# abiswas-odu/Disco

Measured on AMD Instinct MI355X. Metric: overlaps/sec (BuildGraph stage), 150 bp reads, higher is better.
Workload: dtype u64; 1 GPU; 50000000 x 150 bp synthetic reads, 30x of 50 x 5000000 bp uniform-random contigs, both strands, error-free, min-overlap 40 (k=39), transitive reduction on, seed 42; reads=50000000, read_len=150, min_overlap=40, parallelism=1 GPU, e_pre=903537181, e_out=45314794, n_contained=4685156, cap_bind_sites=0, asymmetric_pairs=0, probes=5550000000, kmer_hits=2220071992

## Files before the change

disco_amd/buildgraph.py:

```python
from __future__ import annotations

import ctypes as C
import os

import numpy as np

_HERE = os.path.dirname(os.path.abspath(__file__))
_LIBPATH = os.environ.get("DISCO_LIB") or os.path.join(_HERE, "libdisco_hip.so")
_lib = None


class DiscoError(RuntimeError):
    pass


class Params(C.Structure):
    _fields_ = [("min_overlap", C.c_uint32), ("max_edges_per_kmer", C.c_uint32), ("flags", C.c_uint32), ("max_substitutions", C.c_uint32)]


class GenSpecABI(C.Structure):
    _fields_ = [("seed", C.c_uint64), ("n_reads", C.c_uint64), ("contig_len", C.c_uint64), ("n_contigs", C.c_uint32),
                ("len_min", C.c_uint32), ("len_max", C.c_uint32), ("skew", C.c_uint32)]


# ... 59 lines not shown
    ("disco_contract_chains", C.c_int, [_P, C.c_uint32, C.POINTER(C.c_uint64), C.POINTER(C.c_uint64)]),
    ("disco_contract_chains_of", C.c_int, [_P, _P, C.c_uint64, C.c_uint32, C.POINTER(C.c_uint64), C.POINTER(C.c_uint64)]),
    ("disco_fetch_chains", C.c_int, [_P, _P, _P, _P]),
    ("disco_set_query_order", C.c_int, [_P, _P]),
    ("disco_get_query_order", C.c_int, [_P, C.POINTER(_P)]),
    ("disco_probe_run_words", C.c_int, [_P]),
    ("disco_measure_hbm", C.c_int, [_P, C.c_uint64, C.c_int, C.POINTER(C.c_double)]),
    ("disco_measure_gather", C.c_int, [_P, C.c_uint64, C.c_int, C.POINTER(C.c_double)]),
    ("disco_comm_unique_id", C.c_int, [_P, C.c_size_t]),
    ("disco_comm_init", C.c_int, [_P, _P, C.c_int, C.c_int]),
    ("disco_comm_init_local", C.c_int, [C.POINTER(_P), C.c_int]),
    ("disco_comm_rank", C.c_int, [_P]),
    ("disco_comm_world", C.c_int, [_P]),
    ("disco_comm_kind", C.c_char_p, [_P]),
    ("disco_dist_range", C.c_int, [_P, C.c_uint64, C.POINTER(C.c_uint64), C.POINTER(C.c_uint64)]),
    ("disco_dist_upload_reads", C.c_int, [_P, _P, C.c_uint32, _P, C.c_uint64]),
    ("disco_dist_generate_reads", C.c_int, [_P, C.POINTER(GenSpecABI)]),
    ("disco_dist_run_graph", C.c_int, [_P, C.c_uint32]),
    ("disco_dist_get_info", C.c_int, [_P, _P]),
    ("disco_ingest_fasta", C.c_int, [_P, C.POINTER(C.c_char_p), C.c_int, C.c_uint32, _P, _P]),
    ("disco_ingest_fetch", C.c_int, [_P, _P, _P]),
]

ABI_VERSION = 2
FLAG_TWO_PASS_VERIFY = 1
XCHG = ("reads", "index_records", "index_shards", "contain", "row_requests", "row_data", "push", "adjacency", "twins", "queries", "hits", "keys", "reads_dealt", "contain_keys")
UNIQUE_ID_BYTES = 128
DIST_GATHER_READS = 1
DIST_KEEP_INDEX_PARTITIONED = 2


CHAIN_EDGE_DTYPE = np.dtype([("a", "<u8"), ("b", "<u8"), ("offset", "<u8"), ("orient", "<u4"), ("n_links", "<u4"), ("first_link", "<u8")])
CHAIN_LINK_DTYPE = np.dtype([("to", "<u4"), ("offset", "<u4"), ("orient", "<u4")])


class IngestFile(C.Structure):
    _fields_ = [("first_index", C.c_uint64), ("last_index", C.c_uint64), ("good", C.c_uint64), ("bad", C.c_uint64)]


class IngestInfo(C.Structure):
    _fields_ = [("n_reads", C.c_uint64), ("total_records", C.c_uint64), ("too_long", C.c_uint64), ("stride_words", C.c_uint32), ("shortest", C.c_uint32),
                ("longest", C.c_uint32), ("read_s", C.c_float), ("device_s", C.c_float)]


class DistInfo(C.Structure):
    _fields_ = [("world", C.c_uint32), ("rank", C.c_uint32), ("n_reads", C.c_uint64), ("own_lo", C.c_uint64), ("own_hi", C.c_uint64),
# ... 3 lines not shown
                ("tr_rounds", C.c_uint32), ("tr_deferred", C.c_uint64), ("bytes_sent", C.c_uint64 * len(XCHG)),
                ("ms", C.c_float * len(XCHG)), ("ms_total", C.c_float), ("kernel_ms", C.c_float), ("comm_ops", C.c_uint32),
                ("host_syncs", C.c_uint32), ("device_allocs", C.c_uint32), ("device_frees", C.c_uint32), ("arena_bytes", C.c_uint64),
                ("arena_peak", C.c_uint64), ("hbm_peak", C.c_uint64), ("own_reads", C.c_uint64), ("placement", C.c_uint32), ("reserved_", C.c_uint32)]

PHASES = ("index", "probe_kernel", "verify", "contain", "select", "csr", "twin", "trmark", "emit", "order")


def lib_path() -> str:
    return _LIBPATH


def load():
    global _lib
    if _lib is None:
        if not os.path.exists(_LIBPATH):
            raise DiscoError(f"{_LIBPATH} is missing: build it with `python -m disco_amd.build` (hipcc, gfx950). "
                             "There is no CPU fallback.")
        L = C.CDLL(_LIBPATH)
        L.disco_abi_version.restype = C.c_int
        if L.disco_abi_version() != ABI_VERSION:
            raise DiscoError(f"{_LIBPATH} speaks ABI version {L.disco_abi_version()}, this mirror was written against {ABI_VERSION}: rebuild "
                             "(`python -m disco_amd.build`)")
        for name, res, args in ABI:
            fn = getattr(L, name)
            fn.restype = res
            fn.argtypes = args
        _lib = L
    return _lib


class BuildGraph:

    def __init__(self, min_overlap: int = 40, device: int = 0, max_edges_per_kmer: int = 4, flags: int = 0, max_substitutions: int = 0):
        self.L = load()
        self.min_overlap = min_overlap
        self._h = _P()
        p = Params(min_overlap, max_edges_per_kmer, flags, max_substitutions)
        rc = self.L.disco_create(device, C.byref(p), C.byref(self._h))
        if rc != 0:
            raise DiscoError(f"disco_create failed ({rc}): {self.L.disco_last_error(None).decode()}")

    def _chk(self, rc):
        if rc < 0:
            raise DiscoError(f"libdisco_hip error {rc}: {self.L.disco_last_error(self._h).decode()}")
        return rc

# ... 209 lines not shown

    def fetch_edge_files(self, n_files: int):
        n = int(self.L.disco_fetch_edges(self._h, None, 0))
        out = np.zeros(max(n, 1), dtype=np.uint16)
        self._chk(self.L.disco_fetch_edge_files(self._h, n_files, out.ctypes.data, n))
        return out[:n]

    def partition_edges(self, edges: np.ndarray, n_nodes: int, n_files: int):
        edges = np.ascontiguousarray(edges, dtype=EDGE_DTYPE)
        out = np.zeros(max(len(edges), 1), dtype=np.uint16)
        self._chk(self.L.disco_partition_edges(self._h, edges.ctypes.data, len(edges), n_nodes, n_files, out.ctypes.data))
        return out[:len(edges)]

    def get_query_order(self) -> int:
        out = _P()
        self._chk(self.L.disco_get_query_order(self._h, C.byref(out)))
        return out.value or 0

    def set_query_order(self, d_order_ptr: int):
        self._chk(self.L.disco_set_query_order(self._h, _P(d_order_ptr)))

    def probe_run_words(self) -> int:
        return int(self.L.disco_probe_run_words(self._h))

    def measure_hbm(self, nbytes: int = 4 << 30, reps: int = 5) -> float:
        out = C.c_double(0.0)
        self._chk(self.L.disco_measure_hbm(self._h, nbytes, reps, C.byref(out)))
        return out.value

    def measure_gather(self, nbytes: int = 3 << 30, reps: int = 3) -> float:
        out = C.c_double(0.0)
        self._chk(self.L.disco_measure_gather(self._h, nbytes, reps, C.byref(out)))
        return out.value

    def memcpy_d2d(self, dst_ptr: int, src_ptr: int, nbytes: int):
        self._chk(self.L.disco_memcpy_d2d(self._h, _P(dst_ptr), _P(src_ptr), nbytes))

    @staticmethod
    def comm_unique_id() -> bytes:
        buf = C.create_string_buffer(UNIQUE_ID_BYTES)
        rc = load().disco_comm_unique_id(buf, UNIQUE_ID_BYTES)
        if rc != 0:
            raise DiscoError(f"disco_comm_unique_id failed ({rc})")
        return buf.raw

    def comm_init(self, unique_id: bytes, world: int, rank: int):
# ... 133 lines not shown
```

disco_amd/csrc/disco_device.h:

```cpp
#ifndef DISCO_DEVICE_H_
#define DISCO_DEVICE_H_

#include <hip/hip_runtime.h>
#include <stdint.h>

typedef unsigned long long u64;
typedef unsigned int u32;
typedef unsigned short u16;
typedef unsigned char u8;

#define DISCO_WAVE 64
#define DISCO_NOKEY 0x7FFFFFFFFFFFFFFFull

#define PAY_LEN(p) ((u32)((p)&0x7FFFu))
#define PAY_SUFFIX(p) ((u32)(((p) >> 15) & 1u))
#define PAY_REV(p) ((u32)(((p) >> 16) & 1u))
#define PAY_T(p) ((u32)(((p) >> 17) & 0x3Fu))
#define PAY_ID(p) (((p) >> 23) & 0x7FFFFFFFull)
#define PAY_FP(p) ((u32)((p) >> 54))
#define KEY_FP(key) ((u32)((key)&0x3FFu))
#define PAY_MAKE(key, id, t, rev, suf, len) \
    (((u64)KEY_FP(key) << 54) | ((u64)(id) << 23) | ((u64)(t) << 17) | ((u64)(rev) << 16) | ((u64)(suf) << 15) | (u64)(len))

#define HIT_MAKE(j, id, suf, rev, len) (((u64)(j) << 48) | ((u64)(id) << 17) | ((u64)(suf) << 16) | ((u64)(rev) << 15) | (u64)(len))
// ... 32 lines not shown
    case 2: *orient = 2; *offset = j; break;
    default: *orient = 1; *offset = len1 - (k + j); break;
    }
}

__host__ __device__ __forceinline__ void disco_map_hit(u32 is_suffix, u32 rev, u32 len1, u32 k, u32 j, u32 *orient, u32 *offset)
{
    const u32 same = (is_suffix ^ rev ^ 1u) & 1u;
    *orient = (same << 1) | ((is_suffix ^ 1u) & 1u);
    *offset = same ? j : len1 - (k + j);
}

__host__ __device__ __forceinline__ u32 disco_twin_orient(u32 o) { return o == 0 ? 3u : (o == 3 ? 0u : o); }

__host__ __device__ __forceinline__ u64 disco_hash64(u64 x)
{
    x ^= x >> 33;
    x *= 0xFF51AFD7ED558CCDull;
    x ^= x >> 33;
    x *= 0xC4CEB9FE1A85EC53ull;
    x ^= x >> 33;
    return x;
}

#if defined(__HIPCC__)

__device__ __forceinline__ u64 lane_mask_lt()
{
    u32 l = __lane_id();
    return l ? (~0ull >> (64 - l)) : 0ull;
}
__device__ __forceinline__ u32 rank_below(u64 mask) { return __builtin_amdgcn_mbcnt_hi((u32)(mask >> 32), __builtin_amdgcn_mbcnt_lo((u32)mask, 0u)); }

__device__ __forceinline__ u32 row_prefix_min(u32 x)
{
    u32 y;
    y = (u32)__builtin_amdgcn_update_dpp(-1, (int)x, 0x111, 0xF, 0xF, false);
    x = x < y ? x : y;
    y = (u32)__builtin_amdgcn_update_dpp(-1, (int)x, 0x112, 0xF, 0xF, false);
    x = x < y ? x : y;
    y = (u32)__builtin_amdgcn_update_dpp(-1, (int)x, 0x114, 0xF, 0xF, false);
    x = x < y ? x : y;
    y = (u32)__builtin_amdgcn_update_dpp(-1, (int)x, 0x118, 0xF, 0xF, false);
    return x < y ? x : y;
}
__device__ __forceinline__ u32 row_suffix_min(u32 x)
// ... 259 lines not shown
```

disco_amd/csrc/disco_hip.hip:

```cpp
#include <hip/hip_runtime.h>
#include <rocprofiler-sdk-roctx/roctx.h>

#include <algorithm>
#include <atomic>
#include <chrono>
#include <cstdarg>
#include <cstdio>
#include <cstdlib>
#include <cstring>
#include <fcntl.h>
#include <sys/stat.h>
#include <unistd.h>
#include <string>
#include <memory>
#include <thread>
#include <map>
#include <mutex>
#include <vector>

#include "../../include/disco_hip.h"
#include "../../include/disco_hip_test.h"
#include "disco_kernels.h"
#include "disco_dist.h"

// ... 126 lines not shown
    DevBuf<u16> len_own;
    bool reads_owned = false;
    std::vector<uint16_t> h_len;
    bool h_len_ok = false;
    std::mutex h_len_mu;
    u64 q_lo = 0, q_hi = 0;
    bool two_class = false;
    bool dist_two_class = false;
    u64 job_n_long = 0;
    u32 job_short_max = 0;
    int S_ext = 0;
    u64 n_long = 0;
    DevBuf<u64> d_full;
    DevBuf<u32> d_ovf, d_long_ids;
    u32 max_len_all = 0;
    int tailb = 0;
    DevBuf<u32> d_lpos, d_n_list;
    DevBuf<uint2> d_linfo;
    DevBuf<ulonglong2> d_lmeta;

    u64 T = 0;
    int bshift = 0;
    DevBuf<u32> d_bkt;
    DevBuf<u64> d_ent;
    DevBuf<ulonglong2> d_rec;

    DevBuf<u64> d_tile;
    u64 *d_total = nullptr;

    u64 *d_ctr = nullptr;
    u64 *d_wq = nullptr;
    u64 h_ctr[CTR_COUNT] = {0};

    DevBuf<u64> d_best;
    DevBuf<u64> d_hits;
    u64 hits_used = 0;
    u64 *d_bump = nullptr;
    DevBuf<u64> d_row_start;
    DevBuf<u32> d_row_cnt;
    DevBuf<u64> d_big_list;
    DevBuf<u32> d_big_cnt;
    u32 *d_n_big = nullptr;
    DevBuf<u32> d_runs;
    u64 runs_lo = 0, runs_n = 0;
    int runs_lpr = 0;
    DevBuf<u64> d_slow_list;
// ... 279 lines not shown
template <typename T>
static T *disown(disco_ctx *c, DevBuf<T> &b)
{
    T *p = b.p;
    c->hbm_bytes -= b.cap * sizeof(T);
    b = DevBuf<T>();
    return p;
}

static DiscoView view(const disco_ctx *c)
{
    DiscoView v;
    v.reads = c->d_reads;
    v.len = c->d_len;
    v.n = c->n;
    v.S = c->S;
    v.k = c->k;
    v.m = disco_minimizer_len(c->k);
    if (const char *e = getenv("DISCO_MINIMIZER_LEN")) {
        const int m = atoi(e);
        if (m >= 1 && (m & 1) && m <= v.m && c->k - m <= 63) v.m = m;
    }
    v.bkt = c->d_bkt;
    v.ent = c->d_ent;
    v.bshift = c->bshift;
    v.q_lo = c->q_lo;
    v.q_hi = c->q_hi;
    v.ctr = c->d_ctr;
    v.wq = c->d_wq;
    v.full = c->two_class ? c->d_full : nullptr;
    v.ovf = c->two_class ? c->d_ovf : nullptr;
    v.long_ids = c->two_class ? c->d_long_ids : nullptr;
    v.n_long = c->two_class ? (u32)c->n_long : 0u;
    v.SL = c->two_class ? c->S_ext : 0;
    v.tailb = c->two_class ? c->tailb : 0;
    return v;
}

static OwnSet own_set(const disco_ctx *c)
{
    OwnSet o;
    o.otab = c->loci ? c->d_otab : nullptr;
    o.me = c->comm ? (u32)c->comm->rank : 0u;
    o.lo = c->q_lo;
    o.hi = c->q_hi;
    o.list = c->loci ? c->d_order_own : nullptr;
// ... 69 lines not shown
    hipLaunchKernelGGL((scan_apply_kernel<InT, OutT>), dim3((unsigned)nt), dim3(SCAN_BLOCK), 0, st, in, n, tile.p, out);
    if (write_total) hipLaunchKernelGGL((scan_write_total_kernel<OutT>), dim3(1), dim3(1), 0, st, total, out + n);
    HIPCHK(c, hipGetLastError());
    if (total_host) {
        HIPCHK(c, hipMemcpyAsync(total_host, total, sizeof(u64), hipMemcpyDeviceToHost, st));
        HIPCHK(c, hipStreamSynchronize(st));
    }
    return DISCO_OK;
}

template <typename InT, typename OutT>
static int scan_exclusive(disco_ctx *c, const InT *in, u64 n, OutT *out, bool write_total, u64 *total_host)
{
    return scan_exclusive_on<InT, OutT>(c, c->stream, c->d_tile, c->d_total, in, n, out, write_total, total_host);
}

static void free_graph_state(disco_ctx *c)
{
    if (c->keys_pending) {
        c->keys_pending = false;
        if (c->ev_keys) (void)hipEventSynchronize(c->ev_keys);
    }
    release(c, c->d_bkt);
    release(c, c->d_ent);
    release(c, c->d_rec);
    release(c, c->d_best);
    release(c, c->d_hits);
    release(c, c->d_row_start);
    release(c, c->d_row_cnt);
    release(c, c->d_big_list);
    release(c, c->d_big_cnt);
    release(c, c->d_slow_list);
    release(c, c->d_runs);
    c->runs_n = 0;
    c->runs_lpr = 0;
    release(c, c->d_contained);
    release(c, c->d_cbits);
    release(c, c->d_dropbits);
    release(c, c->d_drop_node);
    release(c, c->d_drop_key);
    release(c, c->d_adj_ref);
    release(c, c->d_adj_own);
    release(c, c->d_adj_spare);
    release(c, c->d_start_tmp);
    release(c, c->d_ocnt);
    release(c, c->d_okey);
// ... 219 lines not shown
{
    IndexCountPlan pl;
    CHK(index_count_plan(c, v, lo, hi, &pl));
    return index_count_chunk<COUNT>(c, v, pl, rec, lo, hi);
}

static int index_begin(disco_ctx *c)
{
    u64 T = 1024;
    int logT = 10;
    double tscale = 2.0;
    if (const char *e = getenv("DISCO_BUCKET_SCALE")) tscale = atof(e);
    while ((double)T < tscale * (double)c->n && logT < 32) {
        T <<= 1;
        logT++;
    }
    c->T = T;
    c->bshift = 64 - logT;
    CHK(ensure(c, c->d_bkt, T + 1));
    CHK(ensure(c, c->d_ent, 2 * c->n));
    CHK(ensure(c, c->d_rec, 2 * c->n));
    CHK(ensure(c, c->d_okey, c->n));
    c->adj_imported = false;
    HIPCHK(c, hipMemsetAsync(c->d_bkt, 0, (T + 1) * sizeof(u32), c->stream));
    return DISCO_OK;
}

static int start_contained_rows(disco_ctx *c, bool grouped)
{
    const u64 nc = c->n_contained;
    if (c->crows_pending && c->crows_n == nc && (!grouped || c->cgrp_pending)) return DISCO_OK;
    const bool have_rows = c->crows_pending && c->crows_n == nc;
    if (!have_rows) c->crows_pending = c->cgrp_pending = false;
    const u64 max_rows = getenv("DISCO_EAGER_ROWS_MAX") ? (u64)atoll(getenv("DISCO_EAGER_ROWS_MAX")) : (16ull << 20);
    if (c->comm || nc == 0 || nc > max_rows || c->n >= (1ull << 31)) return DISCO_OK;
    if (!c->aux_stream) {
        HIPCHK(c, hipStreamCreateWithFlags(&c->aux_stream, hipStreamNonBlocking));
        HIPCHK(c, hipEventCreateWithFlags(&c->ev_crows, hipEventDisableTiming));
        HIPCHK(c, hipMalloc((void **)&c->d_total2, sizeof(u64)));
    }
    CHK(ensure(c, c->d_cpos, c->n + 1));
    CHK(ensure_group(c, nc, nc + nc / 4 + 1024, c->d_crow_id, c->d_crow_key, c->d_crow_len));
    if (nc > c->crows_hcap && c->h_ring && !c->crows_in_ring && (u64)c->ring_half * 2 >= (nc + 1024) * 32) {
        if (c->h_crows) (void)hipHostFree(c->h_crows);
        c->h_crows = c->h_ring;
        c->crows_hcap = (u64)c->ring_half * 2 / 32;
        c->crows_in_ring = true;
// ... 1099 lines not shown
int disco_build_index(disco_ctx *c)
{
    DISCO_TRACE("disco_build_index");
    if (!c) return DISCO_E_ARG;
    if (c->phase < 1) return fail(c, DISCO_E_STATE, "disco_build_index: no reads");
    HIPCHK(c, hipSetDevice(c->device));
    ph_begin(c, DISCO_PH_INDEX);
    if (c->index_counted) {
        c->index_counted = false;
    } else {
        CHK(two_class_convert(c));
        CHK(index_begin(c));
        const DiscoView v = view(c);
        IndexCountPlan pl;
        CHK(index_count_plan(c, v, 0, c->n, &pl));
        CHK(index_count_chunk<true>(c, v, pl, c->d_rec, 0, c->n));
        if (c->two_class) {
            const dim3 g((unsigned)((c->n_long + 255) / 256));
            if (c->k > 64) hipLaunchKernelGGL((index_count_kernel<true, true, true>), g, dim3(256), 0, c->stream, v, c->d_bkt, c->d_rec, c->d_okey, (u64)0, c->n_long, pl.ocnt, pl.oslot, pl.oshift);
            else hipLaunchKernelGGL((index_count_kernel<true, false, true>), g, dim3(256), 0, c->stream, v, c->d_bkt, c->d_rec, c->d_okey, (u64)0, c->n_long, pl.ocnt, pl.oslot, pl.oshift);
            HIPCHK(c, hipGetLastError());
        }
    }
    CHK((scan_exclusive<u32, u32>(c, c->d_bkt, c->T + 1, c->d_bkt, false, nullptr)));
    c->order_ready = false;
    if (c->order_counted && c->order_counted_lo == 0 && c->order_counted_hi == c->n && !c->two_class && !getenv("DISCO_NO_ORDERED_FILL")) {
        const u64 order_buckets = 1ull << c->order_counted_bits;
        CHK(ensure(c, c->d_order_own, c->n));
        ph_end(c, DISCO_PH_INDEX);
        ph_begin(c, DISCO_PH_ORDER);
        CHK((scan_exclusive<u32, u32>(c, c->d_ocnt, order_buckets + 1, c->d_ocnt, false, nullptr)));
        hipLaunchKernelGGL(order_scatter_kernel, dim3(flat_grid(c, c->n)), dim3(256), 0, c->stream, c->d_okey, c->d_oslot, c->d_ocnt, 32u - (u32)c->order_counted_bits, (u64)0, c->n, c->d_len, c->d_order_own);
        ph_end(c, DISCO_PH_ORDER);
        ph_begin(c, DISCO_PH_INDEX2);
        hipLaunchKernelGGL(index_fill_ordered_kernel, dim3(flat_grid(c, c->n)), dim3(256), 0, c->stream, c->n, (const u64 *)c->d_order_own, (const ulonglong2 *)c->d_rec, (const u32 *)c->d_bkt, c->d_ent);
        ph_end(c, DISCO_PH_INDEX2);
        HIPCHK(c, hipGetLastError());
        c->order_ready = true;
        c->phase = 2;
        return DISCO_OK;
    }
    if (c->n) hipLaunchKernelGGL(index_fill_kernel, dim3(flat_grid(c, 2 * c->n)), dim3(256), 0, c->stream, 2 * c->n, c->d_rec, c->d_bkt, c->d_ent);
    HIPCHK(c, hipGetLastError());
    ph_end(c, DISCO_PH_INDEX);
    c->phase = 2;
    return DISCO_OK;
}

int disco_probe(disco_ctx *c)
{
    DISCO_TRACE("disco_probe");
    if (!c) return DISCO_E_ARG;
    if (c->phase < 2) return fail(c, DISCO_E_STATE, "disco_probe: build the index first");
    HIPCHK(c, hipSetDevice(c->device));
    CHK(settle_contained_rows(c));
    CHK(settle_keys(c));
    settle_hits_prealloc(c);
    const u64 nq = c->q_hi - c->q_lo;
// ... 1920 lines not shown
    } else if (c->k > 64)
        hipLaunchKernelGGL((index_count_kernel<false, true>), grid, dim3(256), 0, c->stream, v, c->d_bkt, rec, (u32 *)nullptr, (u64)0, n_own, (u32 *)nullptr, (u32 *)nullptr, 0u, list);
    else
        hipLaunchKernelGGL(index_count_kernel<false>, grid, dim3(256), 0, c->stream, v, c->d_bkt, rec, (u32 *)nullptr, (u64)0, n_own, (u32 *)nullptr, (u32 *)nullptr, 0u, list);
    HIPCHK(c, hipGetLastError());
    return DISCO_OK;
}

static int dist_build_index(disco_ctx *c)
{
    DISCO_TRACE("dist_build_index");
    const u32 G = (u32)c->comm->world, r = (u32)c->comm->rank;
    const u64 nloc = c->q_hi - c->q_lo;
    u64 T = 1024;
    int logT = 10;
    double tscale = 2.0;
    if (const char *e = getenv("DISCO_BUCKET_SCALE")) tscale = atof(e);
    while ((double)T < tscale * (double)c->n && logT < 32) {
        T <<= 1;
        logT++;
    }
    c->T = T;
    c->bshift = 64 - logT;
    auto blo_of = [&](u64 g) { return (g * T + G - 1) / G; };
    const u64 blo = blo_of(r), bhi = blo_of(r + 1);
    const bool part = c->part_index;
    if (!part) {
        CHK(ensure(c, c->d_bkt, T + 1));
        CHK(ensure(c, c->d_ent, 2 * c->n));
    }
    CHK(ensure(c, c->d_okey, c->loci ? c->n_alloc : c->n));
    CHK(ensure(c, c->d_rec, std::max<u64>(2 * nloc, 1)));
    c->adj_imported = false;
    ph_begin(c, DISCO_PH_INDEX);
    DiscoView v = view(c);
    if (c->loci) CHK(index_count_own_list(c, v, c->d_rec));
    else {
        IndexCountPlan pl;
        CHK(index_count_plan(c, v, c->q_lo, c->q_hi, &pl));
        CHK(index_count_chunk<false>(c, v, pl, c->d_rec, c->q_lo, c->q_hi));
        if (c->two_class && nloc) {
            u32 xb[2] = {0, (u32)c->n_long};
            HIPCHK(c, hipMemcpyAsync(&xb[0], c->d_ovf + c->q_lo, sizeof(u32), hipMemcpyDeviceToHost, c->stream));
            if (c->q_hi < c->n) HIPCHK(c, hipMemcpyAsync(&xb[1], c->d_ovf + c->q_hi, sizeof(u32), hipMemcpyDeviceToHost, c->stream));
            HIPCHK(c, hipStreamSynchronize(c->stream));
            if (xb[1] > xb[0]) {
// ... 713 lines not shown
    if (rc != DISCO_OK) {
        fail(c, rc, "disco_comm_init: %s %s", cm->err.c_str(), bulk ? bulk->err.c_str() : "");
        delete cm;
        delete bulk;
        return rc;
    }
    return comm_attach(c, cm, bulk);
}

int disco_comm_init_local(disco_ctx *const *ctxs, int nranks)
{
    if (!ctxs || nranks < 1 || nranks > DIST_MAX_WORLD) return DISCO_E_ARG;
    for (int r = 0; r < nranks; r++)
        if (!ctxs[r]) return DISCO_E_ARG;
    auto grp = std::make_shared<LoopGroup>(nranks), grp2 = std::make_shared<LoopGroup>(nranks);
    for (int r = 0; r < nranks; r++) {
        const int rc = comm_attach(ctxs[r], new LoopComm(grp, r), new LoopComm(grp2, r));
        if (rc != DISCO_OK) return rc;
    }
    return DISCO_OK;
}

int disco_probe_run_words(const disco_ctx *c) { return c ? c->runs_lpr : 0; }
int disco_comm_rank(const disco_ctx *c) { return (c && c->comm) ? c->comm->rank : 0; }
int disco_comm_world(const disco_ctx *c) { return (c && c->comm) ? c->comm->world : 1; }
const char *disco_comm_kind(const disco_ctx *c) { return (c && c->comm) ? c->comm->kind() : "none"; }

int disco_dist_range(const disco_ctx *c, uint64_t n_total, uint64_t *lo, uint64_t *hi)
{
    if (!c || !lo || !hi) return DISCO_E_ARG;
    u64 per, l, h;
    dist_range(c, n_total, &per, &l, &h);
    *lo = l;
    *hi = h;
    return DISCO_OK;
}

static int dist_set_reads(disco_ctx *c, u64 n_total, uint32_t dstride)
{
    if (!c->comm) return fail(c, DISCO_E_STATE, "no communicator: call disco_comm_init / disco_comm_init_local first");
    CHK(set_reads_common(c, n_total, dstride));
    u64 per, lo, hi;
    dist_range(c, n_total, &per, &lo, &hi);
    c->per = per;
    c->n_alloc = per * (u64)c->comm->world;
    c->q_lo = c->home_lo = lo;
// ... 320 lines not shown
```

disco_amd/csrc/disco_kernels.h:

```cpp
#ifndef DISCO_KERNELS_H_
#define DISCO_KERNELS_H_

#include "disco_device.h"
#include "readgen.h"

#define PROBE_ROWCAP 512
#define PROBE_SEGW 128
#define PROBE_SEGP (PROBE_SEGW + 64)
#define PROBE_ACAP 32
#define PROBE_CHUNK 4096
#define ES_MID 1024
#define ES_DUPBITS 11
#define ES_DUPTAB (1 << ES_DUPBITS)
#ifndef ES_CAP
#define ES_CAP 256
#endif
#ifndef TR_CAP
#define TR_CAP 256
#endif
#define TR_CAP_SMALL 128
#define VERIFY_SW 8
#define ORDER_BUCKET(key, shift) (((key) * 0x9E3779B1u) >> (shift))
#define SCAN_ITEMS 16
#define SCAN_BLOCK 256
// ... 13 lines not shown
    CTR_RAW_HITS,
    CTR_HITS_NEEDED,
    CTR_OVERFLOW,
    CTR_CAP_SITES,
    CTR_ASYM,
    CTR_N_CONTAINED,
    CTR_BAD_LEN,
    CTR_BIG_ROWS,
    CTR_ES_BIG,
    CTR_TR_BIG,
    CTR_MAX_DEG,
    CTR_MAX_ROW,
    CTR_TW_UP,
    CTR_TW_DOWN,
    CTR_ES_SLOW,
    CTR_ADJ_TOTAL,
    CTR_MAX_LEN,
    CTR_DROPPED,
    CTR_MIN_LEN,
    CTR_DROP_ITEMS,
    CTR_SHORT_MAX,
    CTR_TR_MID,
    CTR_ES_MID,
    CTR_COUNT
};

#define WQ_CHUNK 64
#define ORDER_MAKE(id, l) ((u64)(id) | ((u64)(l) << 32))
#define ORDER_ID(o) ((o) & 0xFFFFFFFFull)
#define ORDER_LEN(o) ((int)((o) >> 32))
__device__ __forceinline__ u32 uniform_u32(u32 x) { return (u32)__builtin_amdgcn_readfirstlane((int)x); }
__device__ __forceinline__ u64 uniform_u64(u64 x)
{
    return ((u64)uniform_u32((u32)(x >> 32)) << 32) | uniform_u32((u32)x);
}

template <u32 CHUNK = WQ_CHUNK>
__device__ __forceinline__ bool wq_grab(u64 *counter, u64 n, u64 &beg, u64 &end)
{
    u64 b = 0;
    if ((threadIdx.x & 63) == 0) b = atomicAdd(counter, (u64)CHUNK);
#ifdef WQ_EXP_SHFL
    b = __shfl(b, 0);
#else
    b = uniform_u64(b);
#endif
// ... 34 lines not shown
            if ((threadIdx.x & 63) == 0) t = atomicAdd((u32 *)&counters[16u * q], 1u);
            b = uniform_u32(t);
        }
        if (b < mine) {
            beg = (u64)(first + b) * CHUNK;
            end = beg + CHUNK < n ? beg + CHUNK : n;
            return true;
        }
        st.qi++;
    }
    return false;
}

struct DiscoView {
    const u64 *reads;
    const u16 *len;
    u64 n;
    int S;
    int k;
    int m;
    const u32 *bkt;
    const u64 *ent;
    int bshift;
    u64 q_lo, q_hi;
    u64 *ctr;
    u64 *wq;
    const u64 *full;
    const u32 *ovf;
    const u32 *long_ids;
    u32 n_long;
    int SL;
    int tailb;
};

struct OwnSet {
    const u8 *otab;
    u32 me;
    u64 lo, hi;
    const u64 *list;
    u64 n_own;
    const u32 *ids;
    __device__ __forceinline__ bool mine(u64 v) const { return otab ? otab[v] == (u8)me : (v >= lo && v < hi); }
    __device__ __forceinline__ u64 count() const { return otab ? n_own : hi - lo; }
    __device__ __forceinline__ u64 node(u64 i) const { return otab ? ORDER_ID(list[i]) : lo + i; }
    __device__ __forceinline__ u64 node_by_id(u64 i) const { return otab ? (u64)ids[i] : lo + i; }
};
// ... 295 lines not shown
#endif
        rec[2 * (i - lo)] = make_ulonglong2((bp << 32) | sp, PAY_MAKE(kp, rid, tp, rp, 0, L));
        rec[2 * (i - lo) + 1] = make_ulonglong2((bs << 32) | ss, PAY_MAKE(ks, rid, ts, rs, 1, L));
    }
    __syncthreads();
#if defined(INDEX_EXP_NORUNS)
    if (tid != 9999u) return;
#endif
    const u64 r0 = (u64)blockIdx.x * 256u;
    const u64 nr = (hi - lo) - r0 < 256u ? (hi - lo) - r0 : 256u;
    u32 *__restrict__ dst = runs + r0 * (CAP / 2);
    for (u32 x = tid; x < (u32)nr * (CAP / 2); x += 256u) dst[x] = ((const u32 *)s_runs)[x];
}

__global__ void index_fill_kernel(u64 n2, const ulonglong2 *__restrict__ rec, const u32 *__restrict__ bkt, u64 *__restrict__ ent)
{
    u64 i = (u64)blockIdx.x * blockDim.x + threadIdx.x;
    for (; i < n2; i += (u64)gridDim.x * blockDim.x) {
        const ulonglong2 r = rec[i];
        ent[(u64)bkt[r.x >> 32] + (u32)r.x] = r.y;
    }
}

__global__ void index_fill_ordered_kernel(u64 nq, const u64 *__restrict__ order, const ulonglong2 *__restrict__ rec, const u32 *__restrict__ bkt, u64 *__restrict__ ent)
{
    u64 i = (u64)blockIdx.x * blockDim.x + threadIdx.x;
    for (; i < nq; i += (u64)gridDim.x * blockDim.x) {
        const u64 id = ORDER_ID(order[i]);
        const ulonglong2 r0 = rec[2 * id], r1 = rec[2 * id + 1];
        ent[(u64)bkt[r0.x >> 32] + (u32)r0.x] = r0.y;
        ent[(u64)bkt[r1.x >> 32] + (u32)r1.x] = r1.y;
    }
}

template <typename InT>
__global__ void __launch_bounds__(SCAN_BLOCK) scan_tile_sums_kernel(const InT *__restrict__ in, u64 n, u64 *__restrict__ tile_sums)
{
    __shared__ u64 s_part[SCAN_BLOCK / DISCO_WAVE];
    u64 base = (u64)blockIdx.x * SCAN_TILE;
    u64 sum = 0;
    for (int i = 0; i < SCAN_ITEMS; i++) {
        u64 idx = base + (u64)i * SCAN_BLOCK + threadIdx.x;
        if (idx < n) sum += (u64)in[idx];
    }
    for (int o = 32; o > 0; o >>= 1) sum += __shfl_down(sum, o);
    if ((threadIdx.x & 63) == 0) s_part[threadIdx.x >> 6] = sum;
    __syncthreads();
    if (threadIdx.x == 0) {
        u64 t = 0;
        for (int w = 0; w < SCAN_BLOCK / DISCO_WAVE; w++) t += s_part[w];
        tile_sums[blockIdx.x] = t;
    }
}

__global__ void __launch_bounds__(1024) scan_sums_kernel(u64 *__restrict__ tile_sums, u64 nt, u64 *__restrict__ total)
{
    __shared__ u64 s_w[16];
    __shared__ u64 s_carry;
    if (threadIdx.x == 0) s_carry = 0;
    __syncthreads();
    for (u64 base = 0; base < nt; base += 1024) {
        u64 idx = base + threadIdx.x;
        u64 x = idx < nt ? tile_sums[idx] : 0;
        u64 incl = x;
        for (int o = 1; o < 64; o <<= 1) {
            u64 y = __shfl_up(incl, o);
            if ((int)(threadIdx.x & 63) >= o) incl += y;
        }
        if ((threadIdx.x & 63) == 63) s_w[threadIdx.x >> 6] = incl;
        __syncthreads();
        u64 woff = 0;
        for (int w = 0; w < (int)(threadIdx.x >> 6); w++) woff += s_w[w];
        u64 carry = s_carry;
        if (idx < nt) tile_sums[idx] = carry + woff + incl - x;
        __syncthreads();
        if (threadIdx.x == 1023) s_carry = carry + woff + incl;
        __syncthreads();
    }
    if (threadIdx.x == 0) *total = s_carry;
}

template <typename InT, typename OutT>
__global__ void __launch_bounds__(SCAN_BLOCK) scan_apply_kernel(const InT *in, u64 n, const u64 *__restrict__ tile_sums, OutT *out)
{
    __shared__ u64 s_w[SCAN_BLOCK / DISCO_WAVE];
    u64 base = (u64)blockIdx.x * SCAN_TILE + (u64)threadIdx.x * SCAN_ITEMS;
    u64 vals[SCAN_ITEMS];
    u64 sum = 0;
#pragma unroll
    for (int i = 0; i < SCAN_ITEMS; i++) {
        u64 idx = base + i;
        vals[i] = idx < n ? (u64)in[idx] : 0;
        sum += vals[i];
    }
    u64 incl = sum;
    for (int o = 1; o < 64; o <<= 1) {
        u64 y = __shfl_up(incl, o);
        if ((int)(threadIdx.x & 63) >= o) incl += y;
    }
    if ((threadIdx.x & 63) == 63) s_w[threadIdx.x >> 6] = incl;
    __syncthreads();
    u64 off = tile_sums[blockIdx.x] + incl - sum;
    for (int w = 0; w < (int)(threadIdx.x >> 6); w++) off += s_w[w];
#pragma unroll
    for (int i = 0; i < SCAN_ITEMS; i++) {
        u64 idx = base + i;
        if (idx < n) out[idx] = (OutT)off;
        off += vals[i];
    }
}

template <typename OutT>
__global__ void scan_write_total_kernel(const u64 *total, OutT *out_n) { *out_n = (OutT)*total; }

struct ProbeRare {
    u64 *bump;
    u64 hits_cap;
    u64 *big_list;
    u32 *big_cnt;
    u32 *n_big;
    u32 big_cap;
    u32 slow_cap;
    u64 *ctr;
    u64 *slow_list;
    u32 *n_slow;
};
struct ProbeArgs {
    DiscoView v;
    u64 *hits;
    u64 *row_start;
    u32 *row_cnt;
// ... 337 lines not shown
}

#ifndef PR_WAVES_PER_SIMD
#define PR_WAVES_PER_SIMD 8
#endif
template <int LPR>
__global__ void __launch_bounds__(64, PR_WAVES_PER_SIMD) probe_runs_kernel(ProbeArgs a, const u32 *__restrict__ runs, u64 runs_lo)
{
    constexpr int G = 64 / LPR;
    constexpr int RS = VERIFY_SW + 1;
    __shared__ u64 s_rows[G * RS];
    __shared__ u32 s_id[G];
    __shared__ u32 s_occ[128];
    __shared__ u32 s_o_fp[64], s_o_start[64], s_o_excl[64], s_o_desc[64];
    __shared__ u8 s_mark[PR_MARKCAP];
#if defined(VERIFY_EXP_HALF)
    __shared__ u32 s_len_exp[G];
#endif
    const u32 lane = threadIdx.x;
    const int k = a.v.k, m = a.v.m, nf = k - m + 1;
    const u32 slot = lane / LPR, e = lane % LPR;
    const u64 le = lane_mask_lt() | (1ull << lane);
    const u64 nq = a.v.q_hi - a.v.q_lo;
    u64 chunk_base = 0;
    u32 chunk_used = PR_CHUNK;
    u32 my_maxrow = 0;
    for (u32 x = lane; x < PR_MARKCAP / 8; x += 64) ((u64 *)s_mark)[x] = 0ull;
    u64 cbeg = 0, cend = 0;
#if defined(WQ_SPLIT_ALL)
    WqSplit wqs;
    while (wq_grab_split(a.v.wq, nq, cbeg, cend, wqs)) {
#else
    while (wq_grab(a.v.wq, nq, cbeg, cend)) {
#endif
        const u64 ci = min(cbeg + lane, cend - 1);
        const u64 ord_chunk = a.order ? a.order[ci] : ORDER_MAKE(a.v.q_lo + ci, a.v.len[a.v.q_lo + ci]);
        if (a.v.full) {
            const bool lng = cbeg + lane < cend && ORDER_LEN(ord_chunk) > DISCO_SHORT_MAX;
            const u64 lm = __ballot(lng);
            if (lm) {
                u32 base = 0;
                if (lane == 0) base = atomicAdd(a.rare->n_slow, (u32)__popcll(lm));
                base = uniform_u32(base);
                if (lng) {
                    const u32 idx = base + rank_below(lm);
                    if (idx < a.rare->slow_cap) a.rare->slow_list[idx] = ORDER_ID(ord_chunk) | ((cbeg + lane) << 32);
// ... 58 lines not shown
            const u32 below = rank_below(m0) + rank_below(m1);
            if (v0) s_occ[below] = OCC_MAKE(slot, e0, wend0);
            if (v1) s_occ[below + 1] = OCC_MAKE(slot, e1, wend1);
            const u32 n_occ = (u32)__popcll(m0) + (u32)__popcll(m1);
            if (sv && e == 0 && myslow && !(a.v.full && LA > DISCO_SHORT_MAX)) {
                const u32 idx = atomicAdd(a.rare->n_slow, 1u);
                if (idx < a.rare->slow_cap) a.rare->slow_list[idx] = (u64)A | (opos << 32);
                else atomicAdd(&a.rare->ctr[CTR_OVERFLOW], 1ull);
                a.meta_ord[opos] = make_ulonglong2(0ull, (u64)LA << 32);
            }
            u32 nrow = 0;
            u32 c_slot[G];
#pragma unroll
            for (int s = 0; s < G; s++) c_slot[s] = 0;
            __syncthreads();
            for (u32 ob = 0; ob < n_occ; ob += 64) {
                const u32 oi = ob + lane;
                u32 d = 0, st = 0, cnt = 0, fp = 0;
                if (oi < n_occ) {
                    d = s_occ[oi];
                    const int prel = (int)OCC_FIRST(d) + (int)OCC_DELTA(d);
                    const u64 key = mmer_key<true>(s_rows + OCC_SLOT(d) * RS, RS, prel, m);
                    const u64 b = key >> a.v.bshift;
                    uint2 se;
#if defined(PR_EXP) && PR_EXP == 3
                    __builtin_memcpy(&se, a.v.bkt + (b & 7u), sizeof se);
                    se.y = se.x + 3u;
#else
                    __builtin_memcpy(&se, a.v.bkt + b, sizeof se);
#endif
                    st = se.x;
                    cnt = se.y - se.x;
                    fp = KEY_FP(key);
                }
                const u32 incl = wave_inclusive_add(cnt);
                const u32 total = (u32)__builtin_amdgcn_readlane((int)incl, 63);
                const u64 nz = __ballot(cnt > 0);
                const u32 nne = (u32)__popcll(nz);
                const u32 excl = incl - cnt;
                __syncthreads();
                if (cnt > 0) {
                    const u32 r = rank_below(nz);
                    s_o_fp[r] = fp;
                    s_o_start[r] = st;
                    s_o_excl[r] = excl;
                    s_o_desc[r] = d;
                    if (excl < PR_MARKCAP) s_mark[excl] = 1;
                }
                __syncthreads();
                const bool marks = total <= PR_MARKCAP;
                u32 nbefore = 0;
                for (u32 base = 0; base < total; base += 64) {
                    const u32 idx = base + lane;
                    const bool in = idx < total;
                    u32 lo;
// ... 3151 lines not shown
```

profiles/make_traffic.py:

```python
#!/usr/bin/env python3
import json
import os
import sys

ROOT = os.path.dirname(os.path.dirname(os.path.abspath(__file__)))
sys.path.insert(0, ROOT)
import bench

src, reads = sys.argv[1], int(sys.argv[2])
pmc = json.load(open(src))
PHASE_OF = {"index_runs_kernel": "index", "index_count_kernel": "index", "index_fill_kernel": "index", "index_fill_ordered_kernel": "index", "scan_tile_sums_kernel": "index", "scan_sums_kernel": "index",
            "scan_apply_kernel": "index", "probe_runs_kernel": "probe_kernel", "probe_kernel": "probe_kernel", "verify_flat_kernel": "verify",
            "verify_kernel": "verify", "contain_flags_kernel": "contain", "edge_select_kernel": "select", "edge_select_flat_kernel": "select", "transitive_mark_kernel": "trmark",
            "emit_half_kernel": "emit", "emit_kernel": "emit"}
phases = {}
for k, v in pmc.items():
    ph = PHASE_OF.get(k.split("<")[0].strip())
    if ph is None:
        continue
    f, w = v.get("FETCH_SIZE", 0.0) * 1024.0, v.get("WRITE_SIZE", 0.0) * 1024.0
    p = phases.setdefault(ph, {"fetch": 0.0, "write": 0.0, "kernels": [], "valu": 0.0, "salu": 0.0, "lds": 0.0, "lds_bank_conflict": 0.0})
    p["fetch"] += f
    p["write"] += w
    p["kernels"].append(k)
    p["valu"] += v.get("SQ_INSTS_VALU", 0.0)
    p["salu"] += v.get("SQ_INSTS_SALU", 0.0)
    p["lds"] += v.get("SQ_INSTS_LDS", 0.0)
    p["lds_bank_conflict"] += v.get("SQ_LDS_BANK_CONFLICT", 0.0)
for p in phases.values():
    p["lo"] = p["fetch"] + p["write"]
    p["hi"] = 2.0 * p["fetch"] + p["write"]
out = {"reads": reads, "gpus": 1, "phases": phases, "kernels_sha16": bench.kernels_sha16(),
       "source": f"{os.path.relpath(src, ROOT)}: FETCH_SIZE, WRITE_SIZE (KB) x 1024 from separate --pmc passes (profiles/prof_pmc.sh) per phase; lo = fetch + "
                 "write, hi = 2 x fetch + write (calibration: gather_rows_kernel reports 1.014 x its known bytes, the streaming copy 0.500 x: the "
                 "hot kernels mix row gathers and streams, the truth lies between)"}
# ... 9 lines not shown
```

Measured before the change: 10.37 billion overlaps/s.

## Add optional compressed bucket directory and coalesce the scan apply kernel

Adds an optional bitmap-plus-rank directory over the bucket offset table. It is built during the exclusive scan and used by the ordered index fill and, optionally, by the probe kernel's bucket lookups. The aim is to shrink the random-access footprint of the bucket table so that lookups hit cache more often. The cost is an extra word fetch and a popcount per lookup. Separately, the generic scan apply kernel is restructured to a wave-strided, coalesced layout using per-item wave scans. The directory is off by default and is enabled only through environment variables.

```diff
diff --git a/disco_amd/buildgraph.py b/disco_amd/buildgraph.py
--- a/disco_amd/buildgraph.py
+++ b/disco_amd/buildgraph.py
@@ -105,6 +105,17 @@
     ("disco_ingest_fetch", C.c_int, [_P, _P, _P]),
 ]
 
+
+
+class BucketDirStat(C.Structure):
+    _fields_ = [(n, C.c_uint64) for n in ("in_use", "probe", "buckets", "n_nonempty", "bytes", "words_copied")]
+
+
+DIR_WORD_DTYPE = np.dtype([("bits", "<u8"), ("rank", "<u4"), ("spare", "<u4")])
+ABI_BY_VALUE = [
+    ("disco_bucket_dir", BucketDirStat, [_P, _P, C.c_uint64]),
+]
+
 ABI_VERSION = 2
 FLAG_TWO_PASS_VERIFY = 1
 XCHG = ("reads", "index_records", "index_shards", "contain", "row_requests", "row_data", "push", "adjacency", "twins", "queries", "hits", "keys", "reads_dealt", "contain_keys")
@@ -154,7 +165,7 @@
         if L.disco_abi_version() != ABI_VERSION:
             raise DiscoError(f"{_LIBPATH} speaks ABI version {L.disco_abi_version()}, this mirror was written against {ABI_VERSION}: rebuild "
                              "(`python -m disco_amd.build`)")
-        for name, res, args in ABI:
+        for name, res, args in ABI + ABI_BY_VALUE:
             fn = getattr(L, name)
             fn.restype = res
             fn.argtypes = args
@@ -410,6 +421,17 @@
 
     def probe_run_words(self) -> int:
         return int(self.L.disco_probe_run_words(self._h))
+
+    def bucket_dir(self, words: bool = False) -> dict:
+        buf = None
+        if words:
+            st = self.L.disco_bucket_dir(self._h, None, 0)
+            buf = np.zeros(max(int(st.buckets) // 64, 1), dtype=DIR_WORD_DTYPE)
+        st = self.L.disco_bucket_dir(self._h, _P(buf.ctypes.data) if buf is not None else None, len(buf) if buf is not None else 0)
+        out = {k: int(getattr(st, k)) for k in ("in_use", "probe", "buckets", "n_nonempty", "bytes")}
+        if words:
+            out["words"] = buf[:int(st.words_copied)]
+        return out
 
     def measure_hbm(self, nbytes: int = 4 << 30, reps: int = 5) -> float:
         out = C.c_double(0.0)
diff --git a/disco_amd/csrc/disco_device.h b/disco_amd/csrc/disco_device.h
--- a/disco_amd/csrc/disco_device.h
+++ b/disco_amd/csrc/disco_device.h
@@ -78,6 +78,60 @@
     x ^= x >> 33;
     return x;
 }
+
+struct alignas(16) BucketDirWord {
+    u32 bits_lo, bits_hi;
+    u32 rank;
+    u32 spare;
+};
+struct alignas(16) BucketDirHeader {
+    u32 use;
+    u32 n_nonempty;
+    u32 spare[2];
+};
+struct BucketTable {
+    const u32 *bkt;
+    const BucketDirWord *words;
+    const u32 *starts;
+};
+
+#if defined(__HIPCC__)
+__device__ __forceinline__ BucketTable disco_bucket_table(const u32 *bkt, const BucketDirHeader *dir, int bshift)
+{
+    BucketTable t;
+    t.bkt = bkt;
+    t.words = nullptr;
+    t.starts = nullptr;
+    if (dir && __builtin_amdgcn_readfirstlane((int)dir->use)) {
+        t.words = (const BucketDirWord *)(dir + 1);
+        t.starts = (const u32 *)(t.words + (1ull << (58 - bshift)));
+    }
+    return t;
+}
+__device__ __forceinline__ void disco_bucket_bounds(const BucketTable &t, u64 b, u32 &start, u32 &count)
+{
+    const u32 *p = t.bkt + b;
+    start = count = 0;
+    if (t.words) {
+        const BucketDirWord w = t.words[b >> 6];
+        const u64 bits = ((u64)w.bits_hi << 32) | w.bits_lo;
+        const u32 i = (u32)b & 63u;
+        if (!((bits >> i) & 1ull)) return;
+        p = t.starts + (w.rank + (u32)__popcll(bits & ((1ull << i) - 1ull)));
+    }
+    uint2 se;
+    __builtin_memcpy(&se, p, sizeof se);
+    start = se.x;
+    count = se.y - se.x;
+}
+__device__ __forceinline__ u32 disco_bucket_start(const BucketTable &t, u64 b)
+{
+    if (!t.words) return t.bkt[b];
+    const BucketDirWord w = t.words[b >> 6];
+    const u64 bits = ((u64)w.bits_hi << 32) | w.bits_lo;
+    return t.starts[w.rank + (u32)__popcll(bits & ((1ull << ((u32)b & 63u)) - 1ull))];
+}
+#endif
 
 #if defined(__HIPCC__)
 
diff --git a/disco_amd/csrc/disco_hip.hip b/disco_amd/csrc/disco_hip.hip
--- a/disco_amd/csrc/disco_hip.hip
+++ b/disco_amd/csrc/disco_hip.hip
@@ -172,6 +172,8 @@
     u64 T = 0;
     int bshift = 0;
     DevBuf<u32> d_bkt;
+    DevBuf<BucketDirHeader> d_bdir;
+    bool dir_active = false, dir_probe = false;
     DevBuf<u64> d_ent;
     DevBuf<ulonglong2> d_rec;
 
@@ -497,6 +499,7 @@
         if (m >= 1 && (m & 1) && m <= v.m && c->k - m <= 63) v.m = m;
     }
     v.bkt = c->d_bkt;
+    v.bdir = c->dir_active && c->dir_probe ? c->d_bdir.p : nullptr;
     v.ent = c->d_ent;
     v.bshift = c->bshift;
     v.q_lo = c->q_lo;
@@ -612,6 +615,8 @@
         if (c->ev_keys) (void)hipEventSynchronize(c->ev_keys);
     }
     release(c, c->d_bkt);
+    release(c, c->d_bdir);
+    c->dir_active = false;
     release(c, c->d_ent);
     release(c, c->d_rec);
     release(c, c->d_best);
@@ -877,7 +882,25 @@
     CHK(ensure(c, c->d_rec, 2 * c->n));
     CHK(ensure(c, c->d_okey, c->n));
     c->adj_imported = false;
+    c->dir_active = false;
     HIPCHK(c, hipMemsetAsync(c->d_bkt, 0, (T + 1) * sizeof(u32), c->stream));
+    return DISCO_OK;
+}
+
+static int scan_buckets_with_directory(disco_ctx *c)
+{
+    const u64 n = c->T + 1, n_words = c->T >> 6, starts_cap = std::min<u64>(c->T, 2 * c->n) + 1;
+    const long long mb = getenv("DISCO_BUCKET_DIR_MAX_MB") ? atoll(getenv("DISCO_BUCKET_DIR_MAX_MB")) : 128;
+    const u64 budget = mb > 0 ? (u64)mb << 20 : 0;
+    const u64 nt = (n + SCAN_TILE - 1) / SCAN_TILE;
+    CHK(ensure(c, c->d_bdir, 1 + n_words + (starts_cap + 3) / 4));
+    CHK(ensure(c, c->d_tile, nt));
+    hipLaunchKernelGGL((scan_tile_sums_kernel<u32, true>), dim3((unsigned)nt), dim3(SCAN_BLOCK), 0, c->stream, (const u32 *)c->d_bkt, n, c->d_tile.p);
+    hipLaunchKernelGGL(scan_sums_kernel, dim3(1), dim3(1024), 0, c->stream, c->d_tile.p, nt, c->d_total);
+    hipLaunchKernelGGL(scan_apply_dir_kernel, dim3((unsigned)nt), dim3(SCAN_BLOCK), 0, c->stream, c->d_bkt.p, n, (const u64 *)c->d_tile.p, c->d_bdir.p, n_words, starts_cap, budget, c->d_ctr);
+    HIPCHK(c, hipGetLastError());
+    c->dir_active = true;
+    c->dir_probe = env_int("DISCO_BUCKET_DIR_PROBE", 0) != 0;
     return DISCO_OK;
 }
 
@@ -2023,9 +2046,13 @@
             HIPCHK(c, hipGetLastError());
         }
     }
-    CHK((scan_exclusive<u32, u32>(c, c->d_bkt, c->T + 1, c->d_bkt, false, nullptr)));
+    const bool ordered_fill = c->order_counted && c->order_counted_lo == 0 && c->order_counted_hi == c->n && !c->two_class && !getenv("DISCO_NO_ORDERED_FILL");
+    c->dir_active = false;
+    const bool dir_wanted = (env_int("DISCO_BUCKET_DIR", 0) != 0 || env_int("DISCO_BUCKET_DIR_PROBE", 0) != 0) && !getenv("DISCO_NO_BUCKET_DIR");
+    if (dir_wanted && ordered_fill && c->n && c->runs_lpr != 0 && !c->comm && c->n < (1ull << 31)) CHK(scan_buckets_with_directory(c));
+    else CHK((scan_exclusive<u32, u32>(c, c->d_bkt, c->T + 1, c->d_bkt, false, nullptr)));
     c->order_ready = false;
-    if (c->order_counted && c->order_counted_lo == 0 && c->order_counted_hi == c->n && !c->two_class && !getenv("DISCO_NO_ORDERED_FILL")) {
+    if (ordered_fill) {
         const u64 order_buckets = 1ull << c->order_counted_bits;
         CHK(ensure(c, c->d_order_own, c->n));
         ph_end(c, DISCO_PH_INDEX);
@@ -2034,7 +2061,8 @@
         hipLaunchKernelGGL(order_scatter_kernel, dim3(flat_grid(c, c->n)), dim3(256), 0, c->stream, c->d_okey, c->d_oslot, c->d_ocnt, 32u - (u32)c->order_counted_bits, (u64)0, c->n, c->d_len, c->d_order_own);
         ph_end(c, DISCO_PH_ORDER);
         ph_begin(c, DISCO_PH_INDEX2);
-        hipLaunchKernelGGL(index_fill_ordered_kernel, dim3(flat_grid(c, c->n)), dim3(256), 0, c->stream, c->n, (const u64 *)c->d_order_own, (const ulonglong2 *)c->d_rec, (const u32 *)c->d_bkt, c->d_ent);
+        hipLaunchKernelGGL(index_fill_ordered_kernel, dim3(flat_grid(c, c->n)), dim3(256), 0, c->stream, c->n, (const u64 *)c->d_order_own, (const ulonglong2 *)c->d_rec, (const u32 *)c->d_bkt,
+                           (const BucketDirHeader *)(c->dir_active ? c->d_bdir.p : nullptr), c->bshift, c->d_ent);
         ph_end(c, DISCO_PH_INDEX2);
         HIPCHK(c, hipGetLastError());
         c->order_ready = true;
@@ -4001,6 +4029,7 @@
     }
     c->T = T;
     c->bshift = 64 - logT;
+    c->dir_active = false;
     auto blo_of = [&](u64 g) { return (g * T + G - 1) / G; };
     const u64 blo = blo_of(r), bhi = blo_of(r + 1);
     const bool part = c->part_index;
@@ -4760,6 +4789,27 @@
 }
 
 int disco_probe_run_words(const disco_ctx *c) { return c ? c->runs_lpr : 0; }
+
+disco_bucket_dir_stat disco_bucket_dir(disco_ctx *c, void *words, uint64_t max_words)
+{
+    disco_bucket_dir_stat o;
+    memset(&o, 0, sizeof o);
+    if (!c) return o;
+    o.buckets = c->T;
+    if (!c->dir_active) return o;
+    const u64 n_words = c->T >> 6;
+    o.in_use = c->h_ctr[CTR_DIR_USE];
+    o.n_nonempty = c->h_ctr[CTR_DIR_NONEMPTY];
+    o.bytes = n_words * sizeof(BucketDirWord) + (o.n_nonempty + 1) * sizeof(u32);
+    o.probe = o.in_use && c->dir_probe ? 1 : 0;
+    if (words && max_words) {
+        const u64 nw = std::min<u64>(max_words, n_words);
+        if (hipSetDevice(c->device) == hipSuccess && hipStreamSynchronize(c->stream) == hipSuccess &&
+            hipMemcpy(words, c->d_bdir.p + 1, nw * sizeof(BucketDirWord), hipMemcpyDeviceToHost) == hipSuccess)
+            o.words_copied = nw;
+    }
+    return o;
+}
 int disco_comm_rank(const disco_ctx *c) { return (c && c->comm) ? c->comm->rank : 0; }
 int disco_comm_world(const disco_ctx *c) { return (c && c->comm) ? c->comm->world : 1; }
 const char *disco_comm_kind(const disco_ctx *c) { return (c && c->comm) ? c->comm->kind() : "none"; }
diff --git a/disco_amd/csrc/disco_kernels.h b/disco_amd/csrc/disco_kernels.h
--- a/disco_amd/csrc/disco_kernels.h
+++ b/disco_amd/csrc/disco_kernels.h
@@ -59,6 +59,8 @@
     CTR_SHORT_MAX,
     CTR_TR_MID,
     CTR_ES_MID,
+    CTR_DIR_USE,
+    CTR_DIR_NONEMPTY,
     CTR_COUNT
 };
 
@@ -139,6 +141,7 @@
     const u32 *bkt;
     const u64 *ent;
     int bshift;
+    const BucketDirHeader *bdir;
     u64 q_lo, q_hi;
     u64 *ctr;
     u64 *wq;
@@ -480,18 +483,20 @@
     }
 }
 
-__global__ void index_fill_ordered_kernel(u64 nq, const u64 *__restrict__ order, const ulonglong2 *__restrict__ rec, const u32 *__restrict__ bkt, u64 *__restrict__ ent)
-{
+__global__ void index_fill_ordered_kernel(u64 nq, const u64 *__restrict__ order, const ulonglong2 *__restrict__ rec, const u32 *__restrict__ bkt, const BucketDirHeader *__restrict__ bdir,
+                                          int bshift, u64 *__restrict__ ent)
+{
+    const BucketTable tab = disco_bucket_table(bkt, bdir, bshift);
     u64 i = (u64)blockIdx.x * blockDim.x + threadIdx.x;
     for (; i < nq; i += (u64)gridDim.x * blockDim.x) {
         const u64 id = ORDER_ID(order[i]);
         const ulonglong2 r0 = rec[2 * id], r1 = rec[2 * id + 1];
-        ent[(u64)bkt[r0.x >> 32] + (u32)r0.x] = r0.y;
-        ent[(u64)bkt[r1.x >> 32] + (u32)r1.x] = r1.y;
-    }
-}
-
-template <typename InT>
+        ent[(u64)disco_bucket_start(tab, r0.x >> 32) + (u32)r0.x] = r0.y;
+        ent[(u64)disco_bucket_start(tab, r1.x >> 32) + (u32)r1.x] = r1.y;
+    }
+}
+
+template <typename InT, bool FLAGS = false>
 __global__ void __launch_bounds__(SCAN_BLOCK) scan_tile_sums_kernel(const InT *__restrict__ in, u64 n, u64 *__restrict__ tile_sums)
 {
     __shared__ u64 s_part[SCAN_BLOCK / DISCO_WAVE];
@@ -499,7 +504,10 @@
     u64 sum = 0;
     for (int i = 0; i < SCAN_ITEMS; i++) {
         u64 idx = base + (u64)i * SCAN_BLOCK + threadIdx.x;
-        if (idx < n) sum += (u64)in[idx];
+        if (idx < n) {
+            const u64 x = (u64)in[idx];
+            sum += FLAGS ? x | ((u64)(x != 0) << 32) : x;
+        }
     }
     for (int o = 32; o > 0; o >>= 1) sum += __shfl_down(sum, o);
     if ((threadIdx.x & 63) == 0) s_part[threadIdx.x >> 6] = sum;
@@ -538,33 +546,101 @@
     if (threadIdx.x == 0) *total = s_carry;
 }
 
+__device__ __forceinline__ u32 scan_wave_inclusive(u32 x) { return wave_inclusive_add(x); }
+__device__ __forceinline__ u64 scan_wave_inclusive(u64 x)
+{
+    const u32 lane = threadIdx.x & 63;
+    for (int o = 1; o < 64; o <<= 1) {
+        const u64 y = __shfl_up(x, o);
+        if ((int)lane >= o) x += y;
+    }
+    return x;
+}
+__device__ __forceinline__ u32 scan_wave_last(u32 x) { return (u32)__builtin_amdgcn_readlane((int)x, 63); }
+__device__ __forceinline__ u64 scan_wave_last(u64 x) { return readlane_u64(x, 63); }
+
 template <typename InT, typename OutT>
 __global__ void __launch_bounds__(SCAN_BLOCK) scan_apply_kernel(const InT *in, u64 n, const u64 *__restrict__ tile_sums, OutT *out)
 {
     __shared__ u64 s_w[SCAN_BLOCK / DISCO_WAVE];
-    u64 base = (u64)blockIdx.x * SCAN_TILE + (u64)threadIdx.x * SCAN_ITEMS;
-    u64 vals[SCAN_ITEMS];
+    const u32 wave = threadIdx.x >> 6, lane = threadIdx.x & 63;
+    const u64 wbase = (u64)blockIdx.x * SCAN_TILE + (u64)wave * (SCAN_ITEMS * DISCO_WAVE);
+    OutT vals[SCAN_ITEMS];
     u64 sum = 0;
 #pragma unroll
     for (int i = 0; i < SCAN_ITEMS; i++) {
-        u64 idx = base + i;
-        vals[i] = idx < n ? (u64)in[idx] : 0;
-        sum += vals[i];
-    }
-    u64 incl = sum;
-    for (int o = 1; o < 64; o <<= 1) {
-        u64 y = __shfl_up(incl, o);
-        if ((int)(threadIdx.x & 63) >= o) incl += y;
-    }
-    if ((threadIdx.x & 63) == 63) s_w[threadIdx.x >> 6] = incl;
+        const u64 idx = wbase + (u64)i * DISCO_WAVE + lane;
+        vals[i] = idx < n ? (OutT)in[idx] : (OutT)0;
+        sum += (u64)vals[i];
+    }
+    for (int o = 32; o > 0; o >>= 1) sum += __shfl_down(sum, o);
+    if (lane == 0) s_w[wave] = sum;
     __syncthreads();
-    u64 off = tile_sums[blockIdx.x] + incl - sum;
-    for (int w = 0; w < (int)(threadIdx.x >> 6); w++) off += s_w[w];
+    u64 carry64 = tile_sums[blockIdx.x];
+    for (u32 w = 0; w < wave; w++) carry64 += s_w[w];
+    OutT carry = (OutT)carry64;
 #pragma unroll
     for (int i = 0; i < SCAN_ITEMS; i++) {
-        u64 idx = base + i;
-        if (idx < n) out[idx] = (OutT)off;
-        off += vals[i];
+        const u64 idx = wbase + (u64)i * DISCO_WAVE + lane;
+        const OutT incl = scan_wave_inclusive(vals[i]);
+        if (idx < n) out[idx] = carry + incl - vals[i];
+        carry += scan_wave_last(incl);
+    }
+}
+
+__global__ void __launch_bounds__(SCAN_BLOCK) scan_apply_dir_kernel(u32 *bkt, u64 n, const u64 *__restrict__ tile_sums, BucketDirHeader *hdr, u64 n_words, u64 starts_cap, u64 budget_bytes,
+                                                                    u64 *__restrict__ ctr)
+{
+    __shared__ u64 s_w[SCAN_BLOCK / DISCO_WAVE];
+    BucketDirWord *words = (BucketDirWord *)(hdr + 1);
+    u32 *starts = (u32 *)(words + n_words);
+    const u32 wave = threadIdx.x >> 6, lane = threadIdx.x & 63;
+    const u64 wbase = (u64)blockIdx.x * SCAN_TILE + (u64)wave * (SCAN_ITEMS * DISCO_WAVE);
+    u32 vals[SCAN_ITEMS];
+    u64 sum = 0;
+#pragma unroll
+    for (int i = 0; i < SCAN_ITEMS; i++) {
+        const u64 idx = wbase + (u64)i * DISCO_WAVE + lane;
+        vals[i] = idx < n ? bkt[idx] : 0u;
+        sum += (u64)vals[i] | ((u64)(vals[i] != 0) << 32);
+    }
+    for (int o = 32; o > 0; o >>= 1) sum += __shfl_down(sum, o);
+    if (lane == 0) s_w[wave] = sum;
+    __syncthreads();
+    u64 carry = tile_sums[blockIdx.x];
+    for (u32 w = 0; w < wave; w++) carry += s_w[w];
+    u32 crec = (u32)carry, cne = (u32)(carry >> 32);
+#pragma unroll
+    for (int i = 0; i < SCAN_ITEMS; i++) {
+        const u64 idx = wbase + (u64)i * DISCO_WAVE + lane;
+        const u32 cnt = vals[i];
+        const u32 incl = wave_inclusive_add(cnt);
+        const u64 bits = __ballot(cnt != 0);
+        const u32 first = crec + incl - cnt;
+        const u64 r = (u64)cne + rank_below(bits);
+        if (idx < n) bkt[idx] = first;
+        if (cnt != 0 && r < starts_cap) starts[r] = first;
+        if (lane == 0 && (idx >> 6) < n_words) {
+            BucketDirWord w;
+            w.bits_lo = (u32)bits;
+            w.bits_hi = (u32)(bits >> 32);
+            w.rank = cne;
+            w.spare = 0;
+            words[idx >> 6] = w;
+        }
+        if (idx == n - 1) {
+            const u64 nne = r + (cnt != 0);
+            if (nne < starts_cap) starts[nne] = first + cnt;
+            BucketDirHeader h;
+            h.use = (nne < starts_cap && n_words * sizeof(BucketDirWord) + (nne + 1) * sizeof(u32) <= budget_bytes) ? 1u : 0u;
+            h.n_nonempty = (u32)nne;
+            h.spare[0] = h.spare[1] = 0;
+            *hdr = h;
+            ctr[CTR_DIR_USE] = h.use;
+            ctr[CTR_DIR_NONEMPTY] = nne;
+        }
+        crec += (u32)__builtin_amdgcn_readlane((int)incl, 63);
+        cne += (u32)__popcll(bits);
     }
 }
 
@@ -948,6 +1024,7 @@
     const u32 slot = lane / LPR, e = lane % LPR;
     const u64 le = lane_mask_lt() | (1ull << lane);
     const u64 nq = a.v.q_hi - a.v.q_lo;
+    const BucketTable tab = disco_bucket_table(a.v.bkt, a.v.bdir, a.v.bshift);
     u64 chunk_base = 0;
     u32 chunk_used = PR_CHUNK;
     u32 my_maxrow = 0;
@@ -1052,15 +1129,14 @@
                     const int prel = (int)OCC_FIRST(d) + (int)OCC_DELTA(d);
                     const u64 key = mmer_key<true>(s_rows + OCC_SLOT(d) * RS, RS, prel, m);
                     const u64 b = key >> a.v.bshift;
+#if defined(PR_EXP) && PR_EXP == 3
                     uint2 se;
-#if defined(PR_EXP) && PR_EXP == 3
                     __builtin_memcpy(&se, a.v.bkt + (b & 7u), sizeof se);
-                    se.y = se.x + 3u;
+                    st = se.x;
+                    cnt = 3u;
 #else
-                    __builtin_memcpy(&se, a.v.bkt + b, sizeof se);
-#endif
-                    st = se.x;
-                    cnt = se.y - se.x;
+                    disco_bucket_bounds(tab, b, st, cnt);
+#endif
                     fp = KEY_FP(key);
                 }
                 const u32 incl = wave_inclusive_add(cnt);
diff --git a/profiles/make_traffic.py b/profiles/make_traffic.py
--- a/profiles/make_traffic.py
+++ b/profiles/make_traffic.py
@@ -10,7 +10,7 @@
 src, reads = sys.argv[1], int(sys.argv[2])
 pmc = json.load(open(src))
 PHASE_OF = {"index_runs_kernel": "index", "index_count_kernel": "index", "index_fill_kernel": "index", "index_fill_ordered_kernel": "index", "scan_tile_sums_kernel": "index", "scan_sums_kernel": "index",
-            "scan_apply_kernel": "index", "probe_runs_kernel": "probe_kernel", "probe_kernel": "probe_kernel", "verify_flat_kernel": "verify",
+            "scan_apply_kernel": "index", "scan_apply_dir_kernel": "index", "probe_runs_kernel": "probe_kernel", "probe_kernel": "probe_kernel", "verify_flat_kernel": "verify",
             "verify_kernel": "verify", "contain_flags_kernel": "contain", "edge_select_kernel": "select", "edge_select_flat_kernel": "select", "transitive_mark_kernel": "trmark",
             "emit_half_kernel": "emit", "emit_kernel": "emit"}
 phases = {}
```

New measurement: 10.49 billion overlaps/s (median of 6 runs). Within noise of the previous version (+1.2%).
